# HybridRobotics/car-racing

Hardware: AMD Instinct MI355X
Metric: NLP solves/sec (N=12, 6-state bicycle); p50 per-step solve latency (higher is better)
Workload: dtype f64

## Files before the change

car-racing_amd/csrc/crx_kernels.hip:

```cpp
#include <hip/hip_runtime.h>
#include <math.h>
#include <stdint.h>
#include <type_traits>

#include "crx_kparams.h"
#include "crx_wave.h"
#include "crx_num.h"
#include "crx_ipm.h"

#ifndef CRX_TU_GENERAL
#define CRX_TU_GENERAL 0
#endif
#ifndef CRX_TU_MODELS
#define CRX_TU_MODELS 0
#endif
#if CRX_TU_GENERAL
#ifndef CRX_ROWDPP
#define CRX_ROWDPP 0
#endif
#ifndef CRX_OPAQUE_LANE
#define CRX_OPAQUE_LANE 2
#endif
#ifndef CRX_SWEEP_LOCAL_LANE
#define CRX_SWEEP_LOCAL_LANE 0
#endif
#endif
#if CRX_TU_MODELS
using crx_solve_params = crx_kparams_models;
#else
using crx_solve_params = crx_kparams;
#endif
constexpr bool MODELS = CRX_TU_MODELS != 0;
#ifndef CRX_OPAQUE_LANE
#define CRX_OPAQUE_LANE 1
#endif
#ifndef CRX_STATIC_LDS
#define CRX_STATIC_LDS 1
#endif
#ifndef CRX_SWEEP_MASK
#define CRX_SWEEP_MASK 1
#endif
#ifndef CRX_SWEEP_LOCAL_LANE
#define CRX_SWEEP_LOCAL_LANE 1
#endif
#define MAXF 12

__device__ __forceinline__ double ipow_d(double a, int p) {
    const double a2 = a * a;
    const int h = p >> 1;
    double r = sel(p & 1, a, 1.0);
    r = sel(h >= 1, r * a2, r);
    r = sel(h >= 2, r * a2, r);
    r = sel(h >= 3, r * a2, r);
    r = sel(h >= 4, r * a2, r);
    asm volatile("" : "+v"(r));
    return r;
}

#define ROWS(j, jv, lane_, m_) _Pragma("unroll") for (int q_ = 0; q_ < (L::MR + WAVE - 1) / WAVE; q_++) \
    if (const bool jv = (lane_) + q_ * WAVE < (m_); true) if (const int j = jv ? (lane_) + q_ * WAVE : 0; true)

#define COORDS(e, ev, lane_, n_) _Pragma("unroll") for (int q_ = 0; q_ < (L::NV + WAVE - 1) / WAVE; q_++) \
    if (const bool ev = (lane_) + q_ * WAVE < (n_); true) if (const int e = ev ? (lane_) + q_ * WAVE : 0; true)

#define SINK(cond, off) seli((cond), (off), L::dmy)
#define CBF_ROWS(j, k, ob, ev, lane_, n_) _Pragma("unroll") for (int q_ = 0; q_ < (NMAX * NOBS + WAVE - 1) / WAVE; q_++) \
    if (const bool ev = (lane_) + q_ * WAVE < (n_) * NOBS; true) if (const int e_ = ev ? (lane_) + q_ * WAVE : 0; true) \
    if (const int k = e_ / L::NO; true) if (const int ob = e_ - k * L::NO; true) if (const int j = k * NR + 8 + NOBS + ob; true)
#define ROW_LOADS_DONE() do { if (NOBS == 0) __builtin_amdgcn_sched_barrier(0); } while (0)
#define ROW_IS_CBF(j, n_) (NOBS > 0 && (j) < (n_) * NR && (j) % NR >= 8 + NOBS)
#define LOADS_DONE() __builtin_amdgcn_sched_barrier(0)
#ifndef CRX_LOADS_FIRST
#define CRX_LOADS_FIRST 0x3F
#endif
enum : unsigned { LF_ROW_STEP = 1, LF_ROW_TRIAL = 2, LF_ROW_ACCEPT = 4, LF_ACCEPT_Z = 8, LF_FIRST_ORDER = 16, LF_ASSEMBLE = 32 };
template <int NOBS, int NMAX> constexpr unsigned LoadsFirst = (NOBS == 1 && NMAX == 12 && !CRX_TU_GENERAL) ? (unsigned)(CRX_LOADS_FIRST) : 0u;
#ifndef CRX_CBF_CARRY
#define CRX_CBF_CARRY 1
#endif
template <int NOBS, int NMAX> constexpr bool CbfCarry = (CRX_CBF_CARRY) != 0 && NOBS == 1 && NMAX == 12 && !CRX_TU_GENERAL && NMAX * NOBS <= WAVE;
#define STAGE_FENCE() __builtin_amdgcn_sched_barrier(0)

#define RIV_SIMPLE (1 << 13)
#define RIV_NEG (1 << 14)
#define RIV_IDX(pk) ((pk) & 0x1FFF)
#define RIV_SGN(pk) (((pk) & RIV_SIMPLE) ? (((pk) & RIV_NEG) ? -1.0 : 1.0) : 0.0)
#define SH16(si_) ((unsigned short*)((si_) + L::SH_OFF))
#define RIVT(si_, j) ((int)SH16(si_)[L::riv + (j)])
#define UPDP(si_, l_) ((int)SH16(si_)[L::updP + (l_)])
#define VROW(si_) ((typename L::vrow_t*)(SH16(si_) + L::END_S16))

template <int NOBS, int NMAX>
struct Lay {
    static constexpr int NX = 6 + NOBS, NU = 2 + NOBS, NZ = NX + NU, NR = 8 + 2 * NOBS;
    static constexpr int NO = NOBS ? NOBS : 1;
    static constexpr int MR = NMAX * NR + NOBS;
    static constexpr int NV = (NMAX + 1) * NZ;
    static constexpr int M = 0;
    static constexpr int Z = M + NX * NZ;
    static constexpr int dZ = Z + NV;
    static constexpr int xr = dZ + NV;
    static constexpr int wc = xr + (NMAX + 1) * 6;
    static constexpr int obs_s = wc + NMAX;
    static constexpr int obs_e = obs_s + NOBS * (NMAX + 1);
    static constexpr int rt = obs_e + NOBS * (NMAX + 1);
    static constexpr int rnu = rt + MR;
    static constexpr int rc = rnu + MR;
    static constexpr int rdt = rc + MR;
    static constexpr int rtt = rdt + MR;
    static constexpr bool SLIM = NOBS == 3 && NMAX == 20;
    static constexpr int MRS = SLIM ? 0 : MR;
    static constexpr int rsig = rtt + MR;
    static constexpr int rw = rsig + MRS;
    static constexpr int rsc = rw + MRS;
    static constexpr int csc = rsc + MRS;
    static constexpr int rb = csc + (SLIM ? NMAX * NOBS : 0);
    static constexpr int Gpos = rb + MRS;
    static constexpr int Hd = Gpos + (SLIM ? 0 : NMAX * NOBS * 4);
    static constexpr int hg = Hd + NV;
    static constexpr int ga = hg;
    static constexpr int Jc = hg + NV;
    static constexpr int kS = (Jc + NMAX * NOBS * NZ + 1) & ~1;
    static constexpr int kE = kS + 1;
    static constexpr int HS = NZ + 1;
    static constexpr int TS = NZ;
    static constexpr bool PT_ALIAS = NX * NX + NX + NX * TS <= MR, H_ALIAS = NZ * HS <= NV;
    static constexpr int WORK = kS + (NOBS ? 2 * NMAX : 0);
    static constexpr int P = PT_ALIAS ? rdt : WORK;
    static constexpr int pv = P + NX * NX;
    static constexpr int T = pv + NX;
    static constexpr int WORK2 = PT_ALIAS ? WORK : T + NX * TS;
    static constexpr int H = H_ALIAS ? dZ : WORK2;
    static constexpr int Kk = H_ALIAS ? WORK2 : H + NZ * HS;
// ... 462 lines not shown
        h += ((iss0 && k == 0 && o >= c.nobs) || (iss1 && o >= c.nobs)) ? 1.0 : 0.0;
        int rl, rh;
        coord_rows<L>(si, c, e, k, a, rl, rh);
        const int il = rl >= 0 ? rl : 0, ih = rh >= 0 ? rh : 0;
        double sgl, sgh, wl, wh;
        if constexpr (L::SLIM) {
            sgl = LD(L::rnu + il) * LD(L::rtt + il); wl = LD(L::rdt + il);
            sgh = LD(L::rnu + ih) * LD(L::rtt + ih); wh = LD(L::rdt + ih);
        } else {
            sgl = LD(L::rsig + il); sgh = LD(L::rsig + ih); wl = LD(L::rw + il); wh = LD(L::rw + ih);
        }
        h += sel(rl >= 0, sgl, 0.0) + sel(rh >= 0, sgh, 0.0);
        g += sel(rl >= 0, wl, 0.0) - sel(rh >= 0, wh, 0.0);
        if (NOBS) {
            const int kk = k < N ? k : N - 1;
#pragma unroll
            for (int ob = 0; ob < NOBS; ob++) {
                const int j = kk * L::NR + 8 + NOBS + ob;
                const double csj = cbf_scale<L>(sm, kk, ob);
                const double jca = LD(L::Jc + (kk * L::NO + ob) * L::NZ + a);
                double rsj_, rwj;
                if constexpr (L::SLIM) {
                    rwj = LD(L::rdt + j);
                } else {
                    row_sig_w<L>(sm, j, csj != 0.0, mu, LD(L::rt + j), LD(L::rnu + j), LD(L::rtt + j), LD(L::rc + j), rsj_, rwj);
                    (void)rsj_;
                }
                g += sel(k < N, jca * rwj, 0.0);
                const double cur = LD(L::rnu + j) * csj * c.om * LD(L::G + (kk * L::NO + ob) * 4 + (a == 4 ? 2 : 3));
                h += sel(k < N && (a == 4 || a == 5), cur, 0.0);
            }
        }
        const bool tail = k == N && a >= L::NX;
        LD(L::Hd + e) = sel(tail, 0.0, h);
        LD(SINK(ev, L::hg + e)) = sel(tail, 0.0, g);
    }
    if (NOBS) {
        const int k = c.lane < N ? c.lane : 0;
        double ks = 0.0, ke = 0.0;
#pragma unroll
        for (int o = 0; o < NOBS; o++) {
            const int j = k * L::NR + 8 + NOBS + o;
            const double nd = LD(L::rnu + j) * cbf_scale<L>(sm, k, o);
            ks -= nd * LD(L::G + (k * L::NO + o) * 4 + 0);
            ke -= nd * LD(L::G + (k * L::NO + o) * 4 + 1);
            if constexpr (L::sigS >= 0) LD(L::sigS + k * L::NO + o) = sel(LD(L::csc + k * L::NO + o) != 0.0, LD(L::rnu + j) * LD(L::rtt + j), 0.0);
        }
        LD(L::kS + 2 * k) = ks;
        LD(L::kE + 2 * k) = ke;
    }
    SYNC();
}

template <int NOBS, int NMAX, int UNR = 1, int REG = 0, bool CVX = false, bool KEEPF = false>
__device__ __forceinline__ bool riccati_backward(double* sm, const int* si, const Ctx& c, double dw, long long* tsub = nullptr, bool convex = false) {
    using L = Lay<NOBS, NMAX>;
    constexpr int NX = L::NX, NU = L::NU, NZ = L::NZ, HS = L::HS;
    constexpr int oP = REG ? L::P2 : L::P, opv = REG ? L::pv2 : L::pv, oT = REG ? L::T2 : L::T, oH = REG ? L::H2 : L::H, oKk = REG ? L::Kk2 : L::Kk,
                  okf = REG ? L::kf2 : L::kf, odZ = REG ? L::dZ2 : L::dZ;
    const int N = c.N, lane = c.lane;
    const long long qs = CLK();
    constexpr bool PTR = ROWDPP<L> && L::UCNT == 1 && NX <= 7;
    constexpr bool PREG = !PTR && ROWDPP<L> && L::UCNT == 1;
    constexpr int PVF = (NX * 8) & 15;
    static_assert(!PTR || (NX * 8) / 16 == 3, "p sits in DPP row 3, where hv is formed");
    int lo = lane;
    if constexpr (PTR) asm volatile("" : "+v"(lo));
    const int g8 = lo >> 3, c8 = lo & 7;
    const bool isPm = g8 < NX && c8 < NX, isPv = g8 == NX && c8 < NX;
    double preg = 0.0, pn = 0.0;
    {
        double kSn = NOBS ? LD(L::kS + 2 * (N - 1)) : 0.0, kEn = NOBS ? LD(L::kE + 2 * (N - 1)) : 0.0;
        if constexpr (CVX) { kSn = sel(convex, 0.0, kSn); kEn = sel(convex, 0.0, kEn); }
        kEn += 2.0 * LD(L::wc + N - 1);
        if constexpr (PTR) {
            const double hd = LD(L::Hd + N * NZ + seli(isPm, g8, 0));
            const double hgN = LD(L::hg + N * NZ + seli(c8 < NX, c8, 0));
            pn = sel(isPv, hgN, sel(isPm && g8 == c8, hd + sel(g8 == 4, kSn, sel(g8 == 5, kEn, 0.0)), 0.0));
            if (NOBS) {
                LD(SINK(lo < NX, oT + lo * L::TS + 6)) = 0.0;
                LD(SINK(isPm && c8 == 6, oT + g8 * L::TS + NX + 2)) = pn;
            }
        } else {
#pragma unroll
            for (int q_ = 0; q_ < (NX * NX + WAVE - 1) / WAVE; q_++) {
                const int e0 = lane + q_ * WAVE;
                const int e = e0 < NX * NX ? e0 : 0;
                const int i = e / NX, j = e - i * NX;
                const double hd = LD(L::Hd + N * NZ + i);
                LD(oP + e) = sel(i == j, hd + sel(i == 4, kSn, sel(i == 5, kEn, 0.0)), 0.0);
            }
            const double hgN = LD(L::hg + N * NZ + (lane < NX ? lane : 0));
            LD(SINK(lane < NX, opv + lane)) = hgN;
            preg = hgN;
        }
    }
    SYNC();
    bool ok = true;
    constexpr bool FULL = NZ * NZ <= WAVE;
    constexpr int NTRI = FULL ? NZ * NZ : NZ * (NZ + 1) / 2;
    constexpr int HCNT = (NTRI + WAVE - 1) / WAVE;
    int hr[HCNT], ha[HCNT], hst[HCNT];
#pragma unroll
    for (int q = 0; q < HCNT; q++) {
        const int e0 = lane + q * WAVE;
        const int e = e0 < NTRI ? e0 : 0;
        if (FULL) { hr[q] = e / NZ; ha[q] = e - hr[q] * NZ; }
        else if constexpr (L::SLIM) tri_decode(e, hr[q], ha[q]);
// ... 26 lines not shown
    for (int q = 0; q < HCNT; q++) { m5a[q] = NOBS ? 0.0 : LD(L::M + 5 * NZ + ha[q]); m5r[q] = NOBS ? 0.0 : LD(L::M + 5 * NZ + hr[q]); }
    double mz[NX];
#pragma unroll
    for (int i = 0; i < NX; i++) mz[i] = LD(L::M + i * NZ + lz);
    constexpr int T2CNT = NOBS ? (NX * 2 * NOBS + WAVE - 1) / WAVE : 1;
    int t2ld[T2CNT], t2st[T2CNT];
    bool t2nxt[T2CNT];
#pragma unroll
    for (int q = 0; q < T2CNT; q++) {
        t2ld[q] = oP; t2st[q] = L::dmy; t2nxt[q] = false;
        if (NOBS) {
            const int l2 = lane + q * WAVE;
            const bool v2 = l2 < NX * 2 * NOBS;
            const int e2 = v2 ? l2 : 0;
            const int i2 = e2 / (2 * L::NO), cc = e2 - i2 * (2 * L::NO);
            t2nxt[q] = cc >= NOBS;
            const int o = t2nxt[q] ? cc - NOBS : cc;
            t2ld[q] = oP + i2 * NX + 6 + o;
            t2st[q] = SINK(v2, oT + i2 * L::TS + seli(t2nxt[q], NX + 2 + o, 6 + o));
        }
    }
    constexpr int NP = NX * (NX + 1) / 2 + NX, UCNT = L::UCNT;
    int yiA[UCNT], yjA[UCNT], s0A[UCNT], pst1[UCNT], pst2[UCNT], kstr[UCNT], kstep[UCNT], kst[UCNT];
    bool exSl[UCNT], exEl[UCNT];
    double mSl[UCNT], mEl[UCNT], mdg[HCNT];
#pragma unroll
    for (int q = 0; q < HCNT; q++) mdg[q] = hr[q] == ha[q] ? 1.0 : 0.0;
#pragma unroll
    for (int q = 0; q < UCNT; q++) {
        const int l = lane + q * WAVE;
        int ui, uj; bool isP, isK;
        if constexpr (PTR) {
            isP = isPm || isPv;
            isK = NX == 7 ? c8 == 7 : (g8 == 7 && c8 <= NX);
            ui = seli(isPm, g8 < c8 ? g8 : c8, seli(isPv, c8, 0));
            uj = seli(isPm, g8 < c8 ? c8 : g8, seli(isPv, NX, seli(isK, NX == 7 ? g8 : c8, 0)));
        } else {
            const int upk = UPDP(si, l);
            ui = upk >> 8; uj = upk & 255;
            isP = l < NP; isK = !isP && l < NP + NX + 1;
        }
        const bool gcol = uj >= NX;
        const int ujj = gcol ? NZ : uj;
        yiA[q] = oH + NX * HS + ui; yjA[q] = oH + NX * HS + ujj;
        s0A[q] = FULL ? oH + ui * HS + ujj : seli(gcol, oH + ui * HS + ujj, oH + uj * HS + ui);
        pst1[q] = SINK(isP, seli(gcol, opv + ui, oP + ui * NX + uj));
        pst2[q] = SINK(isP, seli(gcol, opv + ui, oP + uj * NX + ui));
        kstr[q] = seli(isK, seli(gcol, 1, NX), 0); kstep[q] = seli(isK, seli(gcol, NU, NU * NX), 0);
        kst[q] = SINK(isK, seli(gcol, okf, oKk + uj) + (N - 1) * kstep[q]);
        exSl[q] = isP && !gcol && ui == uj && ui == 4; exEl[q] = isP && !gcol && ui == uj && ui == 5;
        mSl[q] = exSl[q] ? 1.0 : 0.0; mEl[q] = exEl[q] ? 1.0 : 0.0;
    }
    if (tsub) tsub[2] += CLK() - qs;
#pragma unroll UNR
    for (int k = N - 1; k >= 0; k--) {
        long long q0 = CLK();
        if constexpr (PTR) {
            __builtin_amdgcn_wave_barrier();
            LD(tst[0]) = halfrow_dot6(pn, mT[0], (lane & 8) != 0);
        } else {
            double pl[TCNT][6];
#pragma unroll
            for (int q = 0; q < TCNT; q++)
#pragma unroll
                for (int j = 0; j < 6; j++) pl[q][j] = LD(tld[q] + j);
            double p2[T2CNT];
#pragma unroll
            for (int q = 0; q < T2CNT; q++) p2[q] = NOBS ? LD(t2ld[q]) : 0.0;
            LOADS_DONE();
#pragma unroll
            for (int q = 0; q < TCNT; q++) {
                double t = 0.0;
#pragma unroll
                for (int j = 0; j < 6; j++) t += pl[q][j] * mT[q][j];
                LD(tst[q]) = t;
            }
            if (NOBS) {
#pragma unroll
                for (int q = 0; q < T2CNT; q++) LD(t2st[q]) = sel(t2nxt[q], p2[q], 0.0);
            }
        }
        SYNC();
        long long q1 = CLK();
        {
            double hvs = LD(L::hg + k * NZ + lz), pvv[NX];
            if constexpr (PTR) __builtin_amdgcn_sched_barrier(0);
            const double kc = (NOBS == 0) ? 2.0 * LD(L::wc + k) : 0.0;
            double tc[HCNT][NX], hd[HCNT], jr[HCNT][L::NO], ja[HCNT][L::NO], rs[L::NO];
#pragma unroll
            for (int q = 0; q < HCNT; q++) {
#pragma unroll
                for (int i = 0; i < NX; i++) tc[q][i] = LD(oT + i * L::TS + ha[q]);
                hd[q] = LD(L::Hd + k * NZ + hr[q]);
                if (NOBS) {
#pragma unroll
                    for (int o = 0; o < NOBS; o++) {
                        jr[q][o] = LD(L::Jc + (k * L::NO + o) * NZ + hr[q]);
                        ja[q][o] = LD(L::Jc + (k * L::NO + o) * NZ + ha[q]);
                    }
                }
            }
            if (NOBS) {
#pragma unroll
                for (int o = 0; o < NOBS; o++) {
                    if constexpr (L::sigS >= 0) {
                        rs[o] = LD(L::sigS + k * L::NO + o);
// ... 74 lines not shown
                rD[j] = frcp(d);
#pragma unroll
                for (int i = j + 1; i < NU; i++) {
                    double u = Lf[i][j];
#pragma unroll
                    for (int q = 0; q < j; q++) u = fma(-Lf[i][q], Cf[j][q], u);
                    Cf[i][j] = u;
                    Lf[i][j] = u * rD[j];
                }
            }
            if constexpr (KEEPF) {
                static_assert(NU * (NU + 1) / 2 <= NZ, "the factor fits the stage's slice of Hd");
                int f_ = 0;
#pragma unroll
                for (int a = 0; a < NU; a++) {
                    LD(SINK(lane == 0, L::Hd + k * NZ + f_)) = rD[a]; f_++;
#pragma unroll
                    for (int b2 = 0; b2 < a; b2++) { LD(SINK(lane == 0, L::Hd + k * NZ + f_)) = Lf[a][b2]; f_++; }
                }
            }
#pragma unroll
            for (int q = 0; q < UCNT; q++) {
#pragma unroll
                for (int a = 1; a < NU; a++) {
#pragma unroll
                    for (int qq = 0; qq < a; qq++) { yi[q][a] -= Lf[a][qq] * yi[q][qq]; yj[q][a] -= Lf[a][qq] * yj[q][qq]; }
                }
#pragma unroll
                for (int a = 0; a < NU; a++) { yj[q][a] *= -rD[a]; t[q] = fma(yi[q][a], yj[q][a], t[q]); }
                t[q] = fma(mSl[q], exS, fma(mEl[q], exE, t[q]));
                if constexpr (PTR) {
                    pn = t[0];
                    if (NOBS) LD(SINK(isPm && c8 == 6, oT + g8 * L::TS + NX + 2)) = pn;
                } else {
                    LD(pst1[q]) = t[q];
                    LD(pst2[q]) = t[q];
                }
                if constexpr (PREG) preg = t[0];
#pragma unroll
                for (int a = NU - 2; a >= 0; a--) {
#pragma unroll
                    for (int qq = a + 1; qq < NU; qq++) yj[q][a] = fma(-Lf[qq][a], yj[q][qq], yj[q][a]);
                }
#pragma unroll
                for (int a = 0; a < NU; a++) LD(kst[q] + a * kstr[q]) = yj[q][a];
                kst[q] -= kstep[q];
            }
        }
        if (!ok) break;
        SYNC();
        long long q4 = CLK();
        if (tsub) { tsub[0] += q1 - q0; tsub[1] += q2 - q1; tsub[3] += q4 - q2; }
    }
    if (!ok) { SYNC(); return false; }
    if constexpr (PTR && NOBS > 0) {
        LD(SINK(isPm, oP + g8 * NX + c8)) = pn;
        LD(SINK(isPv, opv + c8)) = pn;
        SYNC();
    }
    if (lane < NZ) LD(odZ + lane) = 0.0;
    if (NOBS) {
        double Ls[L::NO][L::NO], y[L::NO], Ds[L::NO];
#pragma unroll
        for (int a = 0; a < NOBS; a++) {
#pragma unroll
            for (int b = 0; b <= a; b++) Ls[a][b] = LD(oP + (6 + a) * NX + 6 + b);
            y[a] = -LD(opv + 6 + a);
        }
#pragma unroll
        for (int j = 0; j < NOBS; j++) {
            double d = Ls[j][j];
#pragma unroll
            for (int q = 0; q < j; q++) d -= Ls[j][q] * Ls[j][q] * Ds[q];
            if (!(d > 0.0)) ok = false;
            Ds[j] = d;
#pragma unroll
            for (int i = j + 1; i < NOBS; i++) {
                double t = Ls[i][j];
#pragma unroll
                for (int q = 0; q < j; q++) t -= Ls[i][q] * Ls[j][q] * Ds[q];
                Ls[i][j] = t / d;
            }
        }
        if (ok) {
#pragma unroll
            for (int a = 1; a < NOBS; a++) {
#pragma unroll
                for (int q = 0; q < a; q++) y[a] -= Ls[a][q] * y[q];
            }
#pragma unroll
            for (int a = 0; a < NOBS; a++) y[a] /= Ds[a];
#pragma unroll
            for (int a = NOBS - 2; a >= 0; a--) {
#pragma unroll
                for (int q = a + 1; q < NOBS; q++) y[a] -= Ls[q][a] * y[q];
            }
            SYNC();
            if (lane == 0) {
#pragma unroll
                for (int a = 0; a < NOBS; a++) LD(odZ + 6 + a) = y[a];
            }
        }
    }
    SYNC();
    return ok;
}

template <int NOBS, int NMAX, int UNR = 1>
__device__ __forceinline__ void riccati_backward_vec(double* sm, const Ctx& c) {
    using L = Lay<NOBS, NMAX>;
    static_assert(NOBS == 0 && L::NU == 2, "the second solve exists for the all-linear problems (two inputs per stage)");
    constexpr int NX = L::NX, NU = L::NU, NZ = L::NZ;
    const int N = c.N, lane = c.lane;
    if (!CRX_SWEEP_MASK || lane < NZ) {
        const bool in = CRX_SWEEP_MASK || lane < NZ;
        const int la = in ? lane : 0, lx = la < NX ? la : 0;
        double mcol[NX];
#pragma unroll
        for (int i = 0; i < NX; i++) mcol[i] = LD(L::M + i * NZ + la);
        double p = LD(L::hg + N * NZ + la);
        double gk = LD(L::hg + (N - 1) * NZ + la);
        auto stage = [&](int k) {
            const double gn = LD(L::hg + (k >= 1 ? k - 1 : 0) * NZ + la);
            const double rD0 = LD(L::Hd + k * NZ + 0), rD1 = LD(L::Hd + k * NZ + 1), L10 = LD(L::Hd + k * NZ + 2);
            const double k0 = LD(L::Kk + (k * NU + 0) * NX + lx), k1 = LD(L::Kk + (k * NU + 1) * NX + lx);
            double hv = gk;
            if constexpr (ROWDPP<L>) {
                hv = row_dot<NX, 0>(p, mcol, hv);
            } else {
#pragma unroll
                for (int i = 0; i < NX; i++) hv += mcol[i] * lane_f64(p, i);
            }
            const double hu0 = lane_f64(hv, NX), hu1 = lane_f64(hv, NX + 1);
            const double y1 = hu1 - L10 * hu0;
            const double z1 = y1 * rD1;
            const double z0 = hu0 * rD0 - L10 * z1;
            LD(SINK(in && lane < NU, L::kf + k * NU + lane)) = sel(lane == 0, -z0, -z1);
            p = hv + k0 * hu0 + k1 * hu1;
            gk = gn;
            STAGE_FENCE();
        };
        if constexpr (UNR > 1) {
#pragma unroll UNR
            for (int k = N - 1; k >= 0; k--) stage(k);
        } else {
            for (int k = N - 1; k >= 0; k--) stage(k);
        }
        LD(SINK(in, L::dZ + lane)) = 0.0;
    }
    SYNC();
}

template <int NOBS, int NMAX, int UNR = 1>
__device__ __forceinline__ void riccati_forward(double* sm, const Ctx& c) {
    using L = Lay<NOBS, NMAX>;
// ... 271 lines not shown
}

template <class L>
__device__ __forceinline__ void planner_fallback(double* sm, const crx_kparams& kp, int b, int lane, int N) {
    double* Xb = kp.X + (size_t)b * (N + 1) * 6;
    double* Ub = kp.U + (size_t)b * N * 2;
    const double vx0 = kp.x0[(size_t)b * 6];
    double* bs = sm + L::hg;
    double* be = sm + L::Hd;
    for (int j = lane; j <= N; j += WAVE) {
        bs[j] = kp.bez_s[(size_t)b * (N + 1) + j];
        be[j] = kp.bez_ey[(size_t)b * (N + 1) + j];
    }
    SYNC();
    const double s0 = bs[0];
    for (int e = lane; e < (N + 1) * 6; e += WAVE) {
        const int j = e / 6, i = e - j * 6;
        const double st = s0 + kp.fallback_gain * j * kp.dt_ref * vx0;
        double v = 0.0;
        if (i == 0) v = kp.fallback_gain * vx0;
        else if (i == 4) v = st;
        else if (i == 5) v = interp1d<INTERP_SCAN>(bs, be, N + 1, fmin(fmax(st, bs[0]), bs[N]));
        Xb[e] = v;
    }
    for (int e = lane; e < N * 2; e += WAVE) Ub[e] = 0.0;
    if (lane == 0) kp.cost[b] = INFINITY;
}

#ifndef CRX_PLANNER_WAVES
#define CRX_PLANNER_WAVES 3
#endif
#ifndef CRX_OBS1_WAVES
#define CRX_OBS1_WAVES 2
#endif
#ifndef CRX_KERNEL_EXTRA_ATTR
#define CRX_KERNEL_EXTRA_ATTR
#endif
#ifndef CRX_GEN_WAVES
#define CRX_GEN_WAVES 0
#endif
template <int NOBS, int NMAX> struct MinWaves {
    static constexpr int v = CRX_GEN_WAVES ? CRX_GEN_WAVES : ((NOBS == 1 && NMAX == 12) ? CRX_OBS1_WAVES : ((NOBS == 0 && NMAX == 12) ? CRX_PLANNER_WAVES : 1));
};

template <int NFIX> constexpr int StageUnroll = NFIX == 0 ? 1 : NFIX;
template <int NOBS, int NMAX, int DEG = 0, int NFIX = 0, int SPEC = 0, int QPM = 0>
__global__ void __launch_bounds__(WAVE * (1 + SPEC)) __attribute__((amdgpu_waves_per_eu(MinWaves<NOBS, NMAX>::v))) CRX_KERNEL_EXTRA_ATTR
crx_solve_kernel(const crx_solve_params kp) {
    static_assert(NFIX <= NMAX, "fixed horizon inside the layout");
    using L = Lay<NOBS, NMAX>;
    static_assert(!SPEC || (NOBS > 0 && !L::SLIM && CRX_STATIC_LDS), "the speculating wave exists for the obstacle instantiations of the full, static layout");
    constexpr int NX = L::NX, NZ = L::NZ, NR = L::NR;
    constexpr unsigned LF = (NFIX != 0 && QPM == 0) ? LoadsFirst<NOBS, NMAX> : 0u;
    constexpr bool CBFC = NFIX != 0 && QPM == 0 && CbfCarry<NOBS, NMAX>;
    constexpr int RPASS = (L::MR + WAVE - 1) / WAVE, CPASS = (L::NV + WAVE - 1) / WAVE;
    static_assert(LF == 0 || !L::SLIM, "the loads-first row passes are written for the full layout (row_scale, row_bound, row_sig_w are loads there)");
#if CRX_STATIC_LDS
    __shared__ __attribute__((aligned(16))) double sm[((SPEC ? L::BYTES_SPEC : L::BYTES) + 7) / 8];
#else
    extern __shared__ __attribute__((aligned(16))) double sm[];
#endif
    int* si = (int*)(sm + L::END_D);
    const int lane = SPEC ? (int)(threadIdx.x & (WAVE - 1)) : (int)threadIdx.x, N = NFIX ? NFIX : kp.N;
    if ((int)blockIdx.x >= kp.batch) return;
    const int b = kp.order ? min(max(kp.order[blockIdx.x], 0), kp.batch - 1) : (int)blockIdx.x;
    if (kp.active && kp.active[kp.active_div > 1 ? b / kp.active_div : b] == 0) {
        if (lane == 0) { kp.status[b] = CRX_SKIPPED; kp.iters[b] = 0; }
        return;
    }
    const double *mdl_A = nullptr, *mdl_B = nullptr, *mdl_reach = nullptr;
    const double* mdl_plan = nullptr;
#if CRX_TU_MODELS
    {
        mdl_A = kp.model_A + (size_t)36 * b; mdl_B = kp.model_B + (size_t)12 * b; mdl_reach = kp.model_reach + (size_t)2 * (CRX_MAX_N + 1) * b;
        mdl_plan = kp.model_reach + (size_t)CRX_MAX_N * 7 * b;
        const double v = lane < 36 ? mdl_A[lane] : (lane < 48 ? mdl_B[lane - 36] : 0.0);
        if (__ballot(!isfinite(v)) != 0ull) {
            if (NOBS == 0 && kp.mode == 0) {
                planner_fallback<L>(sm, kp, b, lane, N);
                if (lane == 0) { kp.status[b] = CRX_SINGULAR; kp.kkt[b] = INFINITY; kp.iters[b] = 0; }
                return;
            }
            const double nan = __longlong_as_double(0x7ff8000000000000LL);
            for (int e = lane; e < (N + 1) * 6; e += WAVE) kp.X[(size_t)b * (N + 1) * 6 + e] = nan;
            for (int e = lane; e < N * 2; e += WAVE) kp.U[(size_t)b * N * 2 + e] = nan;
            if (kp.sigma)
                for (int e = lane; e < kp.n_obs_max * (N + 1); e += WAVE) kp.sigma[(size_t)b * kp.n_obs_max * (N + 1) + e] = nan;
            if (lane == 0) { kp.cost[b] = nan; kp.status[b] = CRX_SINGULAR; kp.kkt[b] = INFINITY; kp.iters[b] = 0; }
            return;
        }
    }
#endif
    if (NOBS == 0 && kp.mode == 0 && kp.reach_screen) {
        bool out = false;
        for (int j = lane; j < N; j += WAVE) {
            const double* tab = MODELS ? mdl_plan + j * 7 : nullptr;
            double fr = 0.0;
#pragma unroll
            for (int i = 0; i < 6; i++) fr += (MODELS ? tab[i] : kp.reach_row[j][i]) * kp.x0[(size_t)b * 6 + i];
            const double g = MODELS ? tab[6] : kp.reach_gain[j];
            out = out || kp.ey_lb[(size_t)b * N + j] > fr + g + 1e-6 || kp.ey_ub[b] < fr - g - 1e-6;
        }
        if (__ballot(out) != 0ull) {
            planner_fallback<L>(sm, kp, b, lane, N);
            if (lane == 0) { kp.status[b] = CRX_INFEASIBLE; kp.kkt[b] = INFINITY; kp.iters[b] = 0; }
            return;
        }
    }
    if constexpr (SPEC) {
        if (threadIdx.x >= WAVE) {
            Ctx c1 = {};
            c1.N = N; c1.lane = lane;
            for (;;) {
                __syncthreads();
                const int cmd = __builtin_amdgcn_readfirstlane((int)LD(L::ctl));
                if (cmd == 0) break;
// ... 504 lines not shown
            const double Emu = fmax(e_d, fmax(e_p, e_cm));
            if (ipm_mu_reached(Emu, mu, o.kappa_eps, o.tol)) {
                mu = ipm_next_mu<true>(mu, o.kappa_mu, o.theta_mu, o.tol);
                nf = 0;
            } else
                break;
        }
        const double tau = ipm_tau(mu, o.tau_min);
        long long tc3 = CLK();
        assemble_newton<NOBS, NMAX, LF>(sm, si, c, mu);
        long long tc4 = CLK();
        double dw = 0.0;
        long long tsub[4] = {0, 0, 0, 0};
        bool ok;
        int used_convex = 0;
        if (NOBS && crash && cvx_run > 0 && (cvx_run % CVX_PROBE) != 0) {
            if constexpr (!SPEC) {
                for (int k = lane; k < N; k += WAVE) { LD(L::kS + 2 * k) = 0.0; LD(L::kE + 2 * k) = 0.0; }
                SYNC();
            }
            used_convex = 1;
        }
        if constexpr (SPEC) {
            double sdw = 0.0;
            int cz = used_convex, avail = (crash && !used_convex) ? 1 : 0, tries = 0;
            for (;;) {
                double ndw = sdw;
                int ncz = cz, ntries = tries;
                if (avail) ncz = 1;
                else { ndw = tries == 0 ? (dw_last == 0.0 ? 1e-4 : fmax(1e-20, dw_last / 3.0)) : sdw * (dw_last == 0.0 ? 100.0 : 8.0); ntries = tries + 1; }
                const bool nvalid = !(ndw > 1e40);
                const bool post = nvalid && kp.spec_idle == 0;
                if (lane == 0) { LD(L::ctl) = post ? 1.0 : 2.0; LD(L::ctl + 1) = ndw; LD(L::ctl + 2) = ncz ? 1.0 : 0.0; }
                __syncthreads();
                ok = riccati_backward<NOBS, NMAX, StageUnroll<NFIX>, 0, true>(sm, si, c, sdw, tsub, cz != 0);
                __syncthreads();
                if (ok) { dw = sdw; used_convex = cz; break; }
                dw = ndw;
                if (!nvalid) break;
                if (!post) { sdw = ndw; cz = ncz; avail = 0; tries = ntries; continue; }
                if (__builtin_amdgcn_readfirstlane((int)LD(L::ctl + 3)) != 0) {
                    for (int e = lane; e < N * L::NU * NX; e += WAVE) LD(L::Kk + e) = LD(L::Kk2 + e);
                    for (int e = lane; e < N * L::NU; e += WAVE) LD(L::kf + e) = LD(L::kf2 + e);
                    if (lane < NZ) LD(L::dZ + lane) = LD(L::dZ2 + lane);
                    SYNC();
                    ok = true; used_convex = ncz;
                    break;
                }
                sdw = ntries == 0 ? (dw_last == 0.0 ? 1e-4 : fmax(1e-20, dw_last / 3.0)) : ndw * (dw_last == 0.0 ? 100.0 : 8.0);
                cz = ncz; avail = 0; tries = ntries + 1;
                dw = sdw;
                if (sdw > 1e40) break;
            }
        } else
        for (int tries = 0, convex = (NOBS > 0 && crash && !used_convex) ? 0 : 1;; ) {
            ok = riccati_backward<NOBS, NMAX, StageUnroll<NFIX>>(sm, si, c, dw, tsub);
            if (ok) break;
            if (NOBS && !convex) {
                used_convex = 1;
                convex = 1;
                for (int k = lane; k < N; k += WAVE) { LD(L::kS + 2 * k) = 0.0; LD(L::kE + 2 * k) = 0.0; }
                SYNC();
                continue;
            }
            dw = tries == 0 ? (dw_last == 0.0 ? 1e-4 : fmax(1e-20, dw_last / 3.0)) : dw * (dw_last == 0.0 ? 100.0 : 8.0);
            tries++;
            if (dw > 1e40) break;
        }
        if (!ok) break;
        if (dw != 0.0) dw_last = dw;
        cvx_run = used_convex ? cvx_run + 1 : 0;
        long long tc5 = CLK();
        riccati_forward<NOBS, NMAX, StageUnroll<NFIX>>(sm, c);
        long long tc6 = CLK();
        double rp_max = 0.0, rd_max = 0.0, theta = 0.0, Dphi = 0.0;
        auto row_step_tail = [&](int j, bool cnt, bool store, bool on, double jd, double t, double nu, double rti, double rcj, double rsj, double rwj) {
            const double rp = rcj - t;
            const double dt = sel(on, jd + rp, 0.0);
            const double dnu = sel(on, -rwj + rsj * (rp - dt), 0.0);
            LD(SINK(store, L::rdt + j)) = dt;
            const double dtr = dt * rti;
            rp_max = fmax(rp_max, sel(cnt, -dtr, 0.0));
            rd_max = fmax(rd_max, sel(cnt && on, -dnu * frcp(nu), 0.0));
            theta += sel(cnt && on, fabs(rp), 0.0);
            Dphi -= sel(cnt && on, mu * dtr, 0.0);
        };
        auto row_step = [&](int j, bool cnt, bool store, double sc, double jd) {
            const bool on = sc != 0.0;
            const double t = LD(L::rt + j), nu = LD(L::rnu + j), rti = LD(L::rtt + j), rcj = LD(L::rc + j);
            double rwj, rsj;
            row_sig_w<L>(sm, j, on, mu, t, nu, rti, rcj, rsj, rwj);
            ROW_LOADS_DONE();
            row_step_tail(j, cnt, store, on, jd, t, nu, rti, rcj, rsj, rwj);
        };
        if constexpr ((LF & LF_ROW_STEP) != 0) {
            int pk[RPASS];
            double sc[RPASS], dz[RPASS], t[RPASS], nu[RPASS], rti[RPASS], rcj[RPASS], rsj[RPASS], rwj[RPASS];
            ROWS(j, jv, lane, m) { (void)jv; pk[q_] = RIVT(si, j); }
            __builtin_amdgcn_sched_barrier(0);
            ROWS(j, jv, lane, m) {
                (void)jv;
                sc[q_] = row_scale<L>(sm, si, j, N);
                t[q_] = LD(L::rt + j); nu[q_] = LD(L::rnu + j); rti[q_] = LD(L::rtt + j); rcj[q_] = LD(L::rc + j);
                row_sig_w<L>(sm, j, true, mu, t[q_], nu[q_], rti[q_], rcj[q_], rsj[q_], rwj[q_]);
            }
            __builtin_amdgcn_sched_barrier(0);
// ... 380 lines not shown
```

car-racing_amd/csrc/crx_wave.h:

```cpp
#ifndef CRX_WAVE_H
#define CRX_WAVE_H
#include <hip/hip_runtime.h>
#include <math.h>

#define WAVE 64

__device__ __forceinline__ double wrap_above(double s, double L) {
#pragma unroll 1
    for (int i = 0; i < 4 && s > L && L > 0.0; i++) s -= L;
    if (s > L && L > 0.0 && s < 1e300) { s -= L * (ceil(s / L) - 1.0); if (s > L) s -= L; }
    return s;
}
__device__ __forceinline__ double wrap_below(double s, double L) {
#pragma unroll 1
    for (int i = 0; i < 4 && s < 0.0 && L > 0.0; i++) s += L;
    if (s < 0.0 && L > 0.0 && s > -1e300) { s += L * ceil(-s / L); if (s < 0.0) s += L; }
    return s;
}
#if defined(CRX_SYNC_BARRIER)
#define SYNC() __syncthreads()
#elif defined(CRX_SYNC_FENCE_ONLY)
#define SYNC() __builtin_amdgcn_fence(__ATOMIC_ACQ_REL, "wavefront")
#else
#define SYNC() do { __builtin_amdgcn_fence(__ATOMIC_ACQ_REL, "wavefront"); __builtin_amdgcn_wave_barrier(); } while (0)
#endif

template <int CTRL>
__device__ __forceinline__ double dpp_f64(double v) {
    int lo = __double2loint(v), hi = __double2hiint(v);
    lo = __builtin_amdgcn_update_dpp(lo, lo, CTRL, 0xF, 0xF, false);
    hi = __builtin_amdgcn_update_dpp(hi, hi, CTRL, 0xF, 0xF, false);
    return __hiloint2double(hi, lo);
}
__device__ __forceinline__ double lane_f64(double v, int l) {
    int lo = __builtin_amdgcn_readlane(__double2loint(v), l);
    int hi = __builtin_amdgcn_readlane(__double2hiint(v), l);
    return __hiloint2double(hi, lo);
}
#define CRX_DPPT(i) "v_fmac_f64_dpp %0, %1, %" #i " row_newbcast:%"
#define CRX_DPPE " row_mask:0xf bank_mask:0xf\n\t"
template <int CNT, int FIRST>
__device__ __forceinline__ double row_dot(double x, const double* m, double acc) {
    static_assert(CNT >= 2 && CNT <= 9 && FIRST >= 0 && FIRST + CNT <= 16, "row_newbcast reaches the 16 lanes of a row");
    if constexpr (CNT == 2) asm("s_nop 1\n\t" CRX_DPPT(2) "4" CRX_DPPE CRX_DPPT(3) "5" CRX_DPPE : "+&v"(acc) : "v"(x), "v"(m[0]), "v"(m[1]), "n"(FIRST + 0), "n"(FIRST + 1));
    else if constexpr (CNT == 3) asm("s_nop 1\n\t" CRX_DPPT(2) "5" CRX_DPPE CRX_DPPT(3) "6" CRX_DPPE CRX_DPPT(4) "7" CRX_DPPE : "+&v"(acc) : "v"(x), "v"(m[0]), "v"(m[1]), "v"(m[2]), "n"(FIRST + 0), "n"(FIRST + 1), "n"(FIRST + 2));
    else if constexpr (CNT == 4) asm("s_nop 1\n\t" CRX_DPPT(2) "6" CRX_DPPE CRX_DPPT(3) "7" CRX_DPPE CRX_DPPT(4) "8" CRX_DPPE CRX_DPPT(5) "9" CRX_DPPE : "+&v"(acc) : "v"(x), "v"(m[0]), "v"(m[1]), "v"(m[2]), "v"(m[3]), "n"(FIRST + 0), "n"(FIRST + 1), "n"(FIRST + 2), "n"(FIRST + 3));
    else if constexpr (CNT == 5) asm("s_nop 1\n\t" CRX_DPPT(2) "7" CRX_DPPE CRX_DPPT(3) "8" CRX_DPPE CRX_DPPT(4) "9" CRX_DPPE CRX_DPPT(5) "10" CRX_DPPE CRX_DPPT(6) "11" CRX_DPPE : "+&v"(acc) : "v"(x), "v"(m[0]), "v"(m[1]), "v"(m[2]), "v"(m[3]), "v"(m[4]), "n"(FIRST + 0), "n"(FIRST + 1), "n"(FIRST + 2), "n"(FIRST + 3), "n"(FIRST + 4));
    else if constexpr (CNT == 6) asm("s_nop 1\n\t" CRX_DPPT(2) "8" CRX_DPPE CRX_DPPT(3) "9" CRX_DPPE CRX_DPPT(4) "10" CRX_DPPE CRX_DPPT(5) "11" CRX_DPPE CRX_DPPT(6) "12" CRX_DPPE CRX_DPPT(7) "13" CRX_DPPE : "+&v"(acc) : "v"(x), "v"(m[0]), "v"(m[1]), "v"(m[2]), "v"(m[3]), "v"(m[4]), "v"(m[5]), "n"(FIRST + 0), "n"(FIRST + 1), "n"(FIRST + 2), "n"(FIRST + 3), "n"(FIRST + 4), "n"(FIRST + 5));
    else if constexpr (CNT == 7) asm("s_nop 1\n\t" CRX_DPPT(2) "9" CRX_DPPE CRX_DPPT(3) "10" CRX_DPPE CRX_DPPT(4) "11" CRX_DPPE CRX_DPPT(5) "12" CRX_DPPE CRX_DPPT(6) "13" CRX_DPPE CRX_DPPT(7) "14" CRX_DPPE CRX_DPPT(8) "15" CRX_DPPE : "+&v"(acc) : "v"(x), "v"(m[0]), "v"(m[1]), "v"(m[2]), "v"(m[3]), "v"(m[4]), "v"(m[5]), "v"(m[6]), "n"(FIRST + 0), "n"(FIRST + 1), "n"(FIRST + 2), "n"(FIRST + 3), "n"(FIRST + 4), "n"(FIRST + 5), "n"(FIRST + 6));
    else if constexpr (CNT == 8) asm("s_nop 1\n\t" CRX_DPPT(2) "10" CRX_DPPE CRX_DPPT(3) "11" CRX_DPPE CRX_DPPT(4) "12" CRX_DPPE CRX_DPPT(5) "13" CRX_DPPE CRX_DPPT(6) "14" CRX_DPPE CRX_DPPT(7) "15" CRX_DPPE CRX_DPPT(8) "16" CRX_DPPE CRX_DPPT(9) "17" CRX_DPPE : "+&v"(acc) : "v"(x), "v"(m[0]), "v"(m[1]), "v"(m[2]), "v"(m[3]), "v"(m[4]), "v"(m[5]), "v"(m[6]), "v"(m[7]), "n"(FIRST + 0), "n"(FIRST + 1), "n"(FIRST + 2), "n"(FIRST + 3), "n"(FIRST + 4), "n"(FIRST + 5), "n"(FIRST + 6), "n"(FIRST + 7));
    else if constexpr (CNT == 9) asm("s_nop 1\n\t" CRX_DPPT(2) "11" CRX_DPPE CRX_DPPT(3) "12" CRX_DPPE CRX_DPPT(4) "13" CRX_DPPE CRX_DPPT(5) "14" CRX_DPPE CRX_DPPT(6) "15" CRX_DPPE CRX_DPPT(7) "16" CRX_DPPE CRX_DPPT(8) "17" CRX_DPPE CRX_DPPT(9) "18" CRX_DPPE CRX_DPPT(10) "19" CRX_DPPE : "+&v"(acc) : "v"(x), "v"(m[0]), "v"(m[1]), "v"(m[2]), "v"(m[3]), "v"(m[4]), "v"(m[5]), "v"(m[6]), "v"(m[7]), "v"(m[8]), "n"(FIRST + 0), "n"(FIRST + 1), "n"(FIRST + 2), "n"(FIRST + 3), "n"(FIRST + 4), "n"(FIRST + 5), "n"(FIRST + 6), "n"(FIRST + 7), "n"(FIRST + 8));
    return acc;
}

__device__ __forceinline__ double halfrow_dot6(double x, const double* m, bool upper) {
    double lo = 0.0, hi = 0.0;
#define CRX_HR(i, j, j8) "v_fmac_f64_dpp %0, %2, %" #i " row_newbcast:" #j " row_mask:0xf bank_mask:0xf\n\t" \
                         "v_fmac_f64_dpp %1, %2, %" #i " row_newbcast:" #j8 " row_mask:0xf bank_mask:0xf\n\t"
    asm("s_nop 1\n\t" CRX_HR(3, 0, 8) CRX_HR(4, 1, 9) CRX_HR(5, 2, 10) CRX_HR(6, 3, 11) CRX_HR(7, 4, 12) CRX_HR(8, 5, 13)
        : "+&v"(lo), "+&v"(hi) : "v"(x), "v"(m[0]), "v"(m[1]), "v"(m[2]), "v"(m[3]), "v"(m[4]), "v"(m[5]));
#undef CRX_HR
    return upper ? hi : lo;
}

#define ROW_REDUCE(v, OP)                                                         \
    v = OP(v, dpp_f64<0xB1>(v));                         \
    v = OP(v, dpp_f64<0x4E>(v));                         \
    v = OP(v, dpp_f64<0x141>(v));                        \
    v = OP(v, dpp_f64<0x140>(v));
__device__ __forceinline__ double op_add(double a, double b) { return a + b; }
__device__ __forceinline__ double op_mul(double a, double b) { return a * b; }
__device__ __forceinline__ double op_max(double a, double b) { return fmax(a, b); }
__device__ __forceinline__ double op_min(double a, double b) { return fmin(a, b); }
__device__ __forceinline__ double wave_sum(double v) {
    ROW_REDUCE(v, op_add)
    return (lane_f64(v, 0) + lane_f64(v, 16)) + (lane_f64(v, 32) + lane_f64(v, 48));
}
__device__ __forceinline__ double wave_prod(double v) {
    ROW_REDUCE(v, op_mul)
    return (lane_f64(v, 0) * lane_f64(v, 16)) * (lane_f64(v, 32) * lane_f64(v, 48));
}
__device__ __forceinline__ double wave_max(double v) {
    ROW_REDUCE(v, op_max)
    return fmax(fmax(lane_f64(v, 0), lane_f64(v, 16)), fmax(lane_f64(v, 32), lane_f64(v, 48)));
}
__device__ __forceinline__ double wave_min(double v) {
    ROW_REDUCE(v, op_min)
    return fmin(fmin(lane_f64(v, 0), lane_f64(v, 16)), fmin(lane_f64(v, 32), lane_f64(v, 48)));
}

#if defined(__HIP_DEVICE_COMPILE__) && !defined(__gfx950__)
#error "libcrx targets gfx950 (MI355X / CDNA4) only: crx_wave.h uses v_permlane32_swap / v_permlane16_swap (build with ARCH=gfx950)"
#endif
__device__ __forceinline__ void swap32_f64(double& x, double& y) {
    auto lo = __builtin_amdgcn_permlane32_swap(__double2loint(x), __double2loint(y), false, false);
    auto hi = __builtin_amdgcn_permlane32_swap(__double2hiint(x), __double2hiint(y), false, false);
    x = __hiloint2double(hi[0], lo[0]);
    y = __hiloint2double(hi[1], lo[1]);
}
__device__ __forceinline__ void swap16_f64(double& x, double& y) {
    auto lo = __builtin_amdgcn_permlane16_swap(__double2loint(x), __double2loint(y), false, false);
    auto hi = __builtin_amdgcn_permlane16_swap(__double2hiint(x), __double2hiint(y), false, false);
    x = __hiloint2double(hi[0], lo[0]);
    y = __hiloint2double(hi[1], lo[1]);
}
#define WAVE_REDUCE4(a, b, c, d, OP)                                              \
    do {                                                                          \
        swap32_f64(a, b); double s1_ = OP(a, b);                                  \
        swap32_f64(c, d); double s2_ = OP(c, d);                                  \
        swap16_f64(s1_, s2_); double t_ = OP(s1_, s2_);                           \
        ROW_REDUCE(t_, OP)                                                        \
        a = lane_f64(t_, 0); c = lane_f64(t_, 16); b = lane_f64(t_, 32); d = lane_f64(t_, 48); \
    } while (0)
#define WAVE_REDUCE2(a, b, OP)                                                    \
    do {                                                                          \
        swap32_f64(a, b); double s1_ = OP(a, b), s2_ = s1_;                       \
        swap16_f64(s1_, s2_); double t_ = OP(s1_, s2_);                           \
        ROW_REDUCE(t_, OP)                                                        \
        a = lane_f64(t_, 0); b = lane_f64(t_, 32);                                \
    } while (0)
__device__ __forceinline__ void wave_sum4(double& a, double& b, double& c, double& d) { WAVE_REDUCE4(a, b, c, d, op_add); }
__device__ __forceinline__ void wave_max4(double& a, double& b, double& c, double& d) { WAVE_REDUCE4(a, b, c, d, op_max); }
__device__ __forceinline__ void wave_sum2(double& a, double& b) { WAVE_REDUCE2(a, b, op_add); }
__device__ __forceinline__ void wave_max2(double& a, double& b) { WAVE_REDUCE2(a, b, op_max); }

struct LogAcc {
    double m;
    int e;
    __device__ __forceinline__ LogAcc() : m(1.0), e(0) {}
    __device__ __forceinline__ void mul(double v) {
        int ex;
        m *= frexp(v, &ex);
        e += ex;
    }
    __device__ __forceinline__ double wave_total() {
        return log(wave_prod(m)) + 0.6931471805599453 * wave_sum((double)e);
    }
    __device__ __forceinline__ double wave_total_with(double& other) {
        double ex = (double)e;
        wave_sum2(other, ex);
        return log(wave_prod(m)) + 0.6931471805599453 * ex;
// ... 132 lines not shown
```

Before: 609,000.

## Share Riccati retry setup inside backward pass and streamline wave min/max reductions

The Riccati backward pass can now retry in place. A retry callback either switches to the convex fallback or grows the regularisation, then rebuilds only the terminal P/p registers and restarts the loop through a goto. Before, the caller re-invoked the whole function and repeated the per-lane index setup. Separately, DPP moves now use bound_ctrl with a zero source, and the wave min/max reductions use inline v_max_f64/v_min_f64 asm with scalar operands. This avoids fmax/fmin canonicalisation, at the cost of NaN-handling subtleties. A SPEC lane value is also made opaque to the compiler.

```diff
diff --git a/car-racing_amd/csrc/crx_kernels.hip b/car-racing_amd/csrc/crx_kernels.hip
--- a/car-racing_amd/csrc/crx_kernels.hip
+++ b/car-racing_amd/csrc/crx_kernels.hip
@@ -75,10 +75,15 @@
 #endif
 enum : unsigned { LF_ROW_STEP = 1, LF_ROW_TRIAL = 2, LF_ROW_ACCEPT = 4, LF_ACCEPT_Z = 8, LF_FIRST_ORDER = 16, LF_ASSEMBLE = 32 };
 template <int NOBS, int NMAX> constexpr unsigned LoadsFirst = (NOBS == 1 && NMAX == 12 && !CRX_TU_GENERAL) ? (unsigned)(CRX_LOADS_FIRST) : 0u;
+#ifndef CRX_RETRY_SHARED
+#define CRX_RETRY_SHARED 1
+#endif
 #ifndef CRX_CBF_CARRY
 #define CRX_CBF_CARRY 1
 #endif
-template <int NOBS, int NMAX> constexpr bool CbfCarry = (CRX_CBF_CARRY) != 0 && NOBS == 1 && NMAX == 12 && !CRX_TU_GENERAL && NMAX * NOBS <= WAVE;
+template <int NOBS, int NMAX> constexpr bool Obs1Tuned = NOBS == 1 && NMAX == 12 && !CRX_TU_GENERAL;
+template <int NOBS, int NMAX> constexpr bool RetryShared = (CRX_RETRY_SHARED) != 0 && Obs1Tuned<NOBS, NMAX>;
+template <int NOBS, int NMAX> constexpr bool CbfCarry = (CRX_CBF_CARRY) != 0 && Obs1Tuned<NOBS, NMAX> && NMAX * NOBS <= WAVE;
 #define STAGE_FENCE() __builtin_amdgcn_sched_barrier(0)
 
 #define RIV_SIMPLE (1 << 13)
@@ -647,8 +652,10 @@
     SYNC();
 }
 
-template <int NOBS, int NMAX, int UNR = 1, int REG = 0, bool CVX = false, bool KEEPF = false>
-__device__ __forceinline__ bool riccati_backward(double* sm, const int* si, const Ctx& c, double dw, long long* tsub = nullptr, bool convex = false) {
+struct NoRetry { __device__ __forceinline__ bool operator()(double&) const { return false; } };
+template <int NOBS, int NMAX, int UNR = 1, int REG = 0, bool CVX = false, bool KEEPF = false, bool SHARED = false, class Retry = NoRetry>
+__device__ __forceinline__ bool riccati_backward(double* sm, const int* si, const Ctx& c, double dw, long long* tsub = nullptr, bool convex = false,
+                                                 Retry retry = Retry(), double* dw_used = nullptr) {
     using L = Lay<NOBS, NMAX>;
     constexpr int NX = L::NX, NU = L::NU, NZ = L::NZ, HS = L::HS;
     constexpr int oP = REG ? L::P2 : L::P, opv = REG ? L::pv2 : L::pv, oT = REG ? L::T2 : L::T, oH = REG ? L::H2 : L::H, oKk = REG ? L::Kk2 : L::Kk,
@@ -781,6 +788,12 @@
         mSl[q] = exSl[q] ? 1.0 : 0.0; mEl[q] = exEl[q] ? 1.0 : 0.0;
     }
     if (tsub) tsub[2] += CLK() - qs;
+    int kst0[UCNT];
+    if constexpr (SHARED) {
+#pragma unroll
+        for (int q = 0; q < UCNT; q++) kst0[q] = kst[q];
+    }
+attempt: __attribute__((unused));
 #pragma unroll UNR
     for (int k = N - 1; k >= 0; k--) {
         long long q0 = CLK();
@@ -961,7 +974,10 @@
         long long q4 = CLK();
         if (tsub) { tsub[0] += q1 - q0; tsub[1] += q2 - q1; tsub[3] += q4 - q2; }
     }
-    if (!ok) { SYNC(); return false; }
+    if constexpr (!SHARED) {
+        if (!ok) { SYNC(); return false; }
+    }
+    if (SHARED ? !__any(!ok) : true) {
     if constexpr (PTR && NOBS > 0) {
         LD(SINK(isPm, oP + g8 * NX + c8)) = pn;
         LD(SINK(isPv, opv + c8)) = pn;
@@ -1010,6 +1026,37 @@
                 for (int a = 0; a < NOBS; a++) LD(odZ + 6 + a) = y[a];
             }
         }
+    }
+    }
+    if constexpr (SHARED) {
+        if (__any(!ok)) {
+            SYNC();
+            if (__builtin_amdgcn_readfirstlane((int)retry(dw)) != 0) {
+                static_assert(!SHARED || (PTR && NOBS > 0 && !CVX), "the shared set-up is written for the register-resident (P | p) of the one-obstacle kernel");
+                const long long qt = CLK();
+                int lt = lo;
+                asm volatile("" : "+v"(lt));
+                const int g8t = lt >> 3, c8t = lt & 7;
+                const bool isPmt = g8t < NX && c8t < NX, isPvt = g8t == NX && c8t < NX;
+                const double kSn = LD(L::kS + 2 * (N - 1));
+                double kEn = LD(L::kE + 2 * (N - 1));
+                kEn += 2.0 * LD(L::wc + N - 1);
+                const double hd = LD(L::Hd + N * NZ + seli(isPmt, g8t, 0));
+                const double hgN = LD(L::hg + N * NZ + seli(c8t < NX, c8t, 0));
+                pn = sel(isPvt, hgN, sel(isPmt && g8t == c8t, hd + sel(g8t == 4, kSn, sel(g8t == 5, kEn, 0.0)), 0.0));
+                LD(SINK(lt < NX, oT + lt * L::TS + 6)) = 0.0;
+                LD(SINK(isPmt && c8t == 6, oT + g8t * L::TS + NX + 2)) = pn;
+                SYNC();
+                ok = true;
+#pragma unroll
+                for (int q = 0; q < UCNT; q++) { kst[q] = kst0[q]; asm volatile("" : "+v"(kst[q])); }
+                if (tsub) tsub[2] += CLK() - qt;
+                goto attempt;
+            }
+            *dw_used = dw;
+            return false;
+        }
+        *dw_used = dw;
     }
     SYNC();
     return ok;
@@ -1387,6 +1434,7 @@
     static_assert(!SPEC || (NOBS > 0 && !L::SLIM && CRX_STATIC_LDS), "the speculating wave exists for the obstacle instantiations of the full, static layout");
     constexpr int NX = L::NX, NZ = L::NZ, NR = L::NR;
     constexpr unsigned LF = (NFIX != 0 && QPM == 0) ? LoadsFirst<NOBS, NMAX> : 0u;
+    constexpr bool RSH = NFIX != 0 && QPM == 0 && SPEC == 0 && RetryShared<NOBS, NMAX>;
     constexpr bool CBFC = NFIX != 0 && QPM == 0 && CbfCarry<NOBS, NMAX>;
     constexpr int RPASS = (L::MR + WAVE - 1) / WAVE, CPASS = (L::NV + WAVE - 1) / WAVE;
     static_assert(LF == 0 || !L::SLIM, "the loads-first row passes are written for the full layout (row_scale, row_bound, row_sig_w are loads there)");
@@ -1396,7 +1444,12 @@
     extern __shared__ __attribute__((aligned(16))) double sm[];
 #endif
     int* si = (int*)(sm + L::END_D);
-    const int lane = SPEC ? (int)(threadIdx.x & (WAVE - 1)) : (int)threadIdx.x, N = NFIX ? NFIX : kp.N;
+    int lane_ = SPEC ? (int)(threadIdx.x & (WAVE - 1)) : (int)threadIdx.x;
+    if constexpr (SPEC != 0) {
+        asm volatile("" : "+v"(lane_));
+        __builtin_assume(lane_ >= 0);
+    }
+    const int lane = lane_, N = NFIX ? NFIX : kp.N;
     if ((int)blockIdx.x >= kp.batch) return;
     const int b = kp.order ? min(max(kp.order[blockIdx.x], 0), kp.batch - 1) : (int)blockIdx.x;
     if (kp.active && kp.active[kp.active_div > 1 ? b / kp.active_div : b] == 0) {
@@ -2007,6 +2060,20 @@
                 dw = sdw;
                 if (sdw > 1e40) break;
             }
+        } else if constexpr (RSH) {
+            auto retry = [&](double& dwr) -> bool {
+                if (NOBS && __builtin_amdgcn_readfirstlane((int)(crash && !used_convex)) != 0) {
+                    used_convex = 1;
+                    for (int k = lane; k < N; k += WAVE) { LD(L::kS + 2 * k) = 0.0; LD(L::kE + 2 * k) = 0.0; }
+                    SYNC();
+                    return true;
+                }
+                double dwl = dw_last;
+                asm volatile("" : "+v"(dwl));
+                dwr = dwr == 0.0 ? (dwl == 0.0 ? 1e-4 : fmax(1e-20, dwl / 3.0)) : dwr * (dwl == 0.0 ? 100.0 : 8.0);
+                return !(dwr > 1e40);
+            };
+            ok = riccati_backward<NOBS, NMAX, StageUnroll<NFIX>, 0, false, false, true>(sm, si, c, 0.0, tsub, false, retry, &dw);
         } else
         for (int tries = 0, convex = (NOBS > 0 && crash && !used_convex) ? 0 : 1;; ) {
             ok = riccati_backward<NOBS, NMAX, StageUnroll<NFIX>>(sm, si, c, dw, tsub);
diff --git a/car-racing_amd/csrc/crx_wave.h b/car-racing_amd/csrc/crx_wave.h
--- a/car-racing_amd/csrc/crx_wave.h
+++ b/car-racing_amd/csrc/crx_wave.h
@@ -28,8 +28,8 @@
 template <int CTRL>
 __device__ __forceinline__ double dpp_f64(double v) {
     int lo = __double2loint(v), hi = __double2hiint(v);
-    lo = __builtin_amdgcn_update_dpp(lo, lo, CTRL, 0xF, 0xF, false);
-    hi = __builtin_amdgcn_update_dpp(hi, hi, CTRL, 0xF, 0xF, false);
+    lo = __builtin_amdgcn_update_dpp(0, lo, CTRL, 0xF, 0xF, true);
+    hi = __builtin_amdgcn_update_dpp(0, hi, CTRL, 0xF, 0xF, true);
     return __hiloint2double(hi, lo);
 }
 __device__ __forceinline__ double lane_f64(double v, int l) {
@@ -70,8 +70,10 @@
     v = OP(v, dpp_f64<0x140>(v));
 __device__ __forceinline__ double op_add(double a, double b) { return a + b; }
 __device__ __forceinline__ double op_mul(double a, double b) { return a * b; }
-__device__ __forceinline__ double op_max(double a, double b) { return fmax(a, b); }
-__device__ __forceinline__ double op_min(double a, double b) { return fmin(a, b); }
+__device__ __forceinline__ double op_max(double a, double b) { double r; asm("v_max_f64 %0, %1, %2" : "=v"(r) : "v"(a), "v"(b)); return r; }
+__device__ __forceinline__ double op_min(double a, double b) { double r; asm("v_min_f64 %0, %1, %2" : "=v"(r) : "v"(a), "v"(b)); return r; }
+__device__ __forceinline__ double op_max_sv(double a, double b) { double r; asm("v_max_f64 %0, %1, %2" : "=v"(r) : "s"(a), "v"(b)); return r; }
+__device__ __forceinline__ double op_min_sv(double a, double b) { double r; asm("v_min_f64 %0, %1, %2" : "=v"(r) : "s"(a), "v"(b)); return r; }
 __device__ __forceinline__ double wave_sum(double v) {
     ROW_REDUCE(v, op_add)
     return (lane_f64(v, 0) + lane_f64(v, 16)) + (lane_f64(v, 32) + lane_f64(v, 48));
@@ -82,11 +84,11 @@
 }
 __device__ __forceinline__ double wave_max(double v) {
     ROW_REDUCE(v, op_max)
-    return fmax(fmax(lane_f64(v, 0), lane_f64(v, 16)), fmax(lane_f64(v, 32), lane_f64(v, 48)));
+    return op_max(op_max_sv(lane_f64(v, 0), lane_f64(v, 16)), op_max_sv(lane_f64(v, 32), lane_f64(v, 48)));
 }
 __device__ __forceinline__ double wave_min(double v) {
     ROW_REDUCE(v, op_min)
-    return fmin(fmin(lane_f64(v, 0), lane_f64(v, 16)), fmin(lane_f64(v, 32), lane_f64(v, 48)));
+    return op_min(op_min_sv(lane_f64(v, 0), lane_f64(v, 16)), op_min_sv(lane_f64(v, 32), lane_f64(v, 48)));
 }
 
 #if defined(__HIP_DEVICE_COMPILE__) && !defined(__gfx950__)
```

Result: faster. 618,600 (median of 6 runs) (+1.6%).
